# taqu/cpprcoder

Hardware: AMD Instinct MI355X
Metric: MB/s encode+decode per GPU on 64 KiB blocks; ratio vs CPU ref (higher is better)
Workload: dtype u32

## Files before the change

cpprcoder_amd/csrc/rcx_lane.hpp:

```cpp
#pragma once
#include <stdint.h>

#if defined(__HIPCC__)
#define RCX_DEV __device__ __forceinline__
#define RCX_HD __host__ __device__ inline
#else
#define RCX_HD inline
#define RCX_DEV inline
#define RCX_HOST_SIM 1
#endif

typedef uint8_t u8;
typedef uint32_t u32;
typedef uint64_t u64;
typedef int32_t s32;

struct alignas(16) U4 {
    u32 x, y, z, w;
};

#define RCX_LANES 64
#define RCX_G_L3 0
#define RCX_G_L2 1
#define RCX_G_L1 5
#define RCX_G_L0 21
#define RCX_GROUPS 85
#define RCX_STAGE 64
#define RCX_RING_DW 32
#define RCX_HALVE_AT (1u << 24)

struct alignas(16) DivEntry {
    u32 mul, add, shift, total;
};

#if defined(RCX_HOST_SIM)
RCX_DEV u32 rcx_clz(u32 x) { return (u32)__builtin_clz(x); }
RCX_DEV u32 rcx_mul24(u32 a, u32 b) { return (a & 0xFFFFFFu) * (b & 0xFFFFFFu); }
RCX_DEV u32 rcx_perm(u32 hi, u32 lo, u32 sel)
{
    u64 v = ((u64)hi << 32) | lo;
    u32 out = 0;
    for (int i = 0; i < 4; ++i) out |= (u32)((v >> (8 * ((sel >> (8 * i)) & 7))) & 0xFF) << (8 * i);
    return out;
}
RCX_DEV u32 rcx_bswap(u32 x) { return __builtin_bswap32(x); }
RCX_DEV void rcx_lds_inc(u32* p) { *p += 1; }
#if defined(RCX_SIM_RCP)
RCX_DEV float rcx_rcp(float x) { return RCX_SIM_RCP(1.0f / x); }
#else
RCX_DEV float rcx_rcp(float x) { return 1.0f / x; }
#endif
RCX_DEV bool rcx_any(bool p) { return p; }
RCX_DEV u32 rcx_funnel_shr(u32 hi, u32 lo, u32 sh) { return (u32)(((((u64)hi) << 32) | lo) >> (sh & 31u)); }
#define RCX_COLD inline
extern uint64_t rcx_sim_counters[4];
#define RCX_SIM_COUNT(i, n) (rcx_sim_counters[i] += (n))
#else
#define RCX_SIM_COUNT(i, n) ((void)0)
RCX_DEV u32 rcx_clz(u32 x) { return (u32)__builtin_clz(x); }
RCX_DEV u32 rcx_mul24(u32 a, u32 b) { return __umul24(a, b); }
RCX_DEV u32 rcx_perm(u32 hi, u32 lo, u32 sel) { return __builtin_amdgcn_perm(hi, lo, sel); }
RCX_DEV u32 rcx_bswap(u32 x) { return __builtin_bswap32(x); }
RCX_DEV void rcx_lds_inc(u32* p) { (void)__hip_atomic_fetch_add(p, 1u, __ATOMIC_RELAXED, __HIP_MEMORY_SCOPE_WAVEFRONT); }
RCX_DEV void rcx_lds_add(u32* p, u32 v) { (void)__hip_atomic_fetch_add(p, v, __ATOMIC_RELAXED, __HIP_MEMORY_SCOPE_WAVEFRONT); }
RCX_DEV float rcx_rcp(float x) { return __builtin_amdgcn_rcpf(x); }
RCX_DEV bool rcx_any(bool p) { return __builtin_expect(__any(p) != 0, 0); }
RCX_DEV u32 rcx_funnel_shr(u32 hi, u32 lo, u32 sh) { return __builtin_amdgcn_alignbit(hi, lo, sh); }
#define RCX_COLD __device__ __attribute__((noinline, cold))
#endif

RCX_DEV u32 rcx_div(u32 n, const DivEntry& k) { return (u32)(((u64)n * k.mul + k.add) >> 32) >> k.shift; }

#if !defined(RCX_TREE_PLANAR)
#define RCX_TREE_PLANAR 0
#endif
struct Tree {
    u32* col;
#if RCX_TREE_PLANAR
    RCX_DEV u32* at(u32 g, u32 p) const { return col + (4 * g + p) * RCX_LANES; }
    RCX_DEV U4 group(u32 g) const
    {
        const u32* a = col + 4 * g * RCX_LANES;
        U4 v;
        v.x = a[0];
        v.y = a[RCX_LANES];
        v.z = a[2 * RCX_LANES];
        v.w = a[3 * RCX_LANES];
        return v;
    }
    RCX_DEV void store(u32 g, const U4& v) const
    {
        u32* a = col + 4 * g * RCX_LANES;
        a[0] = v.x;
        a[RCX_LANES] = v.y;
        a[2 * RCX_LANES] = v.z;
        a[3 * RCX_LANES] = v.w;
    }
#else
    RCX_DEV u32* at(u32 g, u32 p) const { return col + 4 * g * RCX_LANES + p; }
    RCX_DEV U4 group(u32 g) const { return *reinterpret_cast<const U4*>(col + 4 * g * RCX_LANES); }
    RCX_DEV void store(u32 g, const U4& v) const { *reinterpret_cast<U4*>(col + 4 * g * RCX_LANES) = v; }
#endif
    RCX_DEV void bump(u32 g, u32 p) const { rcx_lds_inc(at(g, p)); }
    RCX_DEV void put(u32 g, u32 p, u32 value) const { *at(g, p) = value; }
    RCX_DEV void reset() const
    {
        U4 v;
        v.x = v.y = v.z = v.w = 64;
        store(RCX_G_L3, v);
        v.x = v.y = v.z = v.w = 16;
        for (u32 g = RCX_G_L2; g < RCX_G_L1; ++g) store(g, v);
        v.x = v.y = v.z = v.w = 4;
        for (u32 g = RCX_G_L1; g < RCX_G_L0; ++g) store(g, v);
// ... 122 lines not shown
        base = wave_base;
        off = slot_off + 4;
        cap = (slot_bytes - 4) & ~3u;
        reset_state();
    }

    RCX_DEV void idle(u8* wave_base)
    {
        base = wave_base;
        off = 0;
        cap = 0;
        reset_state();
        leader = false;
    }

    RCX_DEV void carry_into_memory(u32 extra) { rcx_carry_walk(base + off, leader ? (pos < cap ? pos : 0u) : 0u, extra); }

    RCX_DEV void track(u32 index, u32 carry, u32 moved, u32 k8)
    {
        if (trk_fail_at != 0xFFFFFFFFu) return;
        if (carry && trk_pending > 0) {
            if (trk_written + trk_pending > trk_cap) { trk_fail_at = index; return; }
            trk_written += trk_pending;
            trk_pending = 0;
        }
        for (u32 s = 0; s < k8; s += 8) {
            if (((moved << s) >> 24) != 0xFFu) {
                if (trk_written + 1 + trk_pending > trk_cap) { trk_fail_at = index; return; }
                trk_written += 1 + trk_pending;
                trk_pending = 0;
            } else {
                trk_pending += 1;
            }
        }
    }
    RCX_DEV bool track_flush_fails() const { return trk_written + 1 + trk_pending > trk_cap; }

    template <bool WIDE = false>
    RCX_DEV u32 arith(u32 cum, u32 f, const DivEntry& k)
    {
        return arith_t<WIDE>(cum, f, rcx_div(range, k));
    }
    template <bool WIDE = false>
    RCX_DEV u32 arith_t(u32 cum, u32 f, u32 t)
    {
        const u32 moved = low + (WIDE ? cum * t : rcx_mul24(cum, t));
        const u32 carry = moved < low ? 1u : 0u;
        range = WIDE ? f * t : rcx_mul24(f, t);
        const u32 k8 = rcx_clz(range) & 0x18u;
        low = moved << k8;
        range <<= k8;
        return (moved & 0xFFFFFF00u) | k8 | carry;
    }
    RCX_DEV u32 arith_q(u32 cum, u32 f, u32 mul, u32 shift, u64 add)
    {
        const u32 t = (u32)(((u64)range * mul + add) >> 32) >> (shift & 31u);
        const u32 moved = low + rcx_mul24(cum, t);
        const u32 carry = moved < low ? 1u : 0u;
        range = rcx_mul24(f, t);
        const u32 k8 = rcx_clz(range) & 0x18u;
        low = moved << k8;
        range <<= k8;
        return (moved & 0xFFFFFF00u) | k8 | carry;
    }
    RCX_DEV void emit(u32 rec)
    {
        const u32 k8 = rec & 0x18u;
        acc += rec & 1u;
        acc = (acc << k8) | (((u64)rec << k8) >> 32);
        nacc8 += k8;
        flush();
    }
    template <bool TRACK = false, bool WIDE = false>
    RCX_DEV void code(u32 cum, u32 f, const DivEntry& k, u32 index = 0)
    {
        const u32 rec = arith<WIDE>(cum, f, k);
        if (TRACK) track(index, rec & 1u, rec & 0xFFFFFF00u, rec & 0x18u);
        emit(rec);
    }

    RCX_DEV void flush()
    {
        const bool due = nacc8 >= 40;
        const u32 keep8 = (nacc8 - 32) & 31u;
        const u32 acc_lo = (u32)acc, acc_hi = (u32)(acc >> 32);
        const u32 word = rcx_funnel_shr(acc_hi, acc_lo, keep8);
        const u32 extra = due ? acc_hi >> keep8 : 0u;
        if (rcx_any(extra != 0)) rcx_carry_slow(base + off, leader ? (pos < cap ? pos : 0u) : 0u, extra);
        const u32 where = pos < cap - 4 ? pos : cap - 4;
        if (due && leader) *reinterpret_cast<u32*>(base + (off + where)) = rcx_bswap(word);
        const u32 kept = acc_lo & ((1u << keep8) - 1u);
        acc = due ? (u64)kept : acc;
        nacc8 -= due ? 32u : 0u;
        pos += due ? 4u : 0u;
    }
    template <bool TRACK = false, class TreeT>
    RCX_DEV void step(const TreeT& tree, u32 c, const DivEntry& k, u32 index = 0)
    {
        const U4 g3 = tree.group(RCX_G_L3);
        const U4 g2 = tree.group(RCX_G_L2 + (c >> 6));
        const U4 g1 = tree.group(RCX_G_L1 + (c >> 4));
        const U4 g0 = tree.group(RCX_G_L0 + (c >> 2));
        const u32 cum = rcx_pre4(g3, c >> 6) + rcx_pre4(g2, (c >> 4) & 3) + rcx_pre4(g1, (c >> 2) & 3) + rcx_pre4(g0, c & 3);
        const u32 f = rcx_sel4(g0, c & 3);
        code<TRACK>(cum, f, k, index);
        tree.update(c);
    }

    template <bool TRACK = false, class TreeT>
    RCX_DEV void step_long(const TreeT& tree, u32 c, u32& total, u32 index = 0)
    {
        const U4 g3 = tree.group(RCX_G_L3);
        const U4 g2 = tree.group(RCX_G_L2 + (c >> 6));
        const U4 g1 = tree.group(RCX_G_L1 + (c >> 4));
        const U4 g0 = tree.group(RCX_G_L0 + (c >> 2));
// ... 319 lines not shown
```

cpprcoder_amd/csrc/rcx_launch.hpp:

```cpp
#pragma once
#include "rcx_ctx.hpp"

namespace
{

bool wide_workgroups(const rcx_ctx* c, u64 nblocks)
{
    (void)nblocks;
    return c->wide_wg != 0;
}

int decode_lanes(const rcx_ctx* c, u64 nblocks)
{
    (void)nblocks;
    return c->lanes_per_block ? c->lanes_per_block : 4;
}

u32 pow2_at_least(u64 x)
{
    u32 p = 1;
    while (p < x) p <<= 1;
    return p;
}
u32 encode_lanes(const rcx_ctx* c, u64 nblocks)
// ... 20 lines not shown
    u32* models;
    u32* redo;
};

template <class G>
int encode_launches(rcx_ctx* c, int coder, const void* d_src, u64 n, u32 block, u64 nblocks, ScratchView v, u64 slot, hipStream_t s, bool packed, G g)
{
    const u8* const src = static_cast<const u8*>(d_src);
    const int variant = (G::items && c->enc_variant != 0) ? 3 : c->enc_variant;
    const bool static3 = coder == RCX_CODER_STATIC && variant >= 2 && nblocks < 32768;
    auto adaptive_pass = [&](const u32* redo) {
        hipLaunchKernelGGL((rcx_enc_adaptive_k<false, false, G>), dim3(grid_for(nblocks, RCX_LANES)), dim3(64), 0, s, src, n, block, nblocks, v.slots,
                           slot, v.sizes, c->divtab(), c->status, 0u, static_cast<u32*>(nullptr), redo, g);
    };
    auto static_pass = [&](const u32* redo) {
        hipLaunchKernelGGL(rcx_enc_static_k<G>, dim3(grid_for(nblocks, RCX_LANES)), dim3(64), 0, s, src, n, block, nblocks, v.slots, slot, v.sizes,
                           c->status, redo, g);
    };
    Timed t(c, s, RCX_T_ENCODE);
    if (is_rans(coder)) {
        const u32 grid = grid_for(nblocks, 4 * RCX_RANS_BLOCKS);
        if (coder == RCX_CODER_RANS8)
            hipLaunchKernelGGL((rcx_enc_rans_k<true, G>), dim3(grid), dim3(256), 0, s, src, n, block, nblocks, v.slots, slot, v.sizes, v.starts,
                               c->status, g);
        else {
            hipLaunchKernelGGL((rcx_rans_model_k<14, G>), dim3(grid), dim3(256), 0, s, src, n, block, nblocks, v.models, g);
            const char* one = getenv("RCX_RANS1_WAVES");
            if (!(one && atoi(one) == 1)) {
                if (allow_lds(c, &rcx_enc_rans1w_k<G>, RCX_R1W_LDS_BYTES) != RCX_OK) return RCX_E_HIP;
                hipLaunchKernelGGL(rcx_enc_rans1w_k<G>, dim3(grid_for(nblocks, 64)), dim3(128), RCX_R1W_LDS_BYTES, s, src, n, block, nblocks,
                                   static_cast<const u32*>(v.models), v.slots, slot, v.sizes, v.starts, c->status, g);
            } else {
                u32 lanes = 16;
                if (const char* v2 = getenv("RCX_RANS1_LANES")) { const int q = atoi(v2); if (q == 1 || q == 2 || q == 4 || q == 8 || q == 16) lanes = (u32)q; }
                u32 lds_bytes = lanes * RCX_RANS1_ENC_WAVES * 2048u;
                if (getenv("RCX_RANS1_ALONE") && lds_bytes < 84u * 1024u) lds_bytes = 84u * 1024u;
                u32 lanes_shift = 0;
                while ((1u << lanes_shift) < lanes) ++lanes_shift;
                if (allow_lds(c, &rcx_enc_rans1_k<G>, 128 * 1024) != RCX_OK) return RCX_E_HIP;
                hipLaunchKernelGGL(rcx_enc_rans1_k<G>, dim3(grid_for(nblocks, (u64)lanes * RCX_RANS1_ENC_WAVES)), dim3(64 * RCX_RANS1_ENC_WAVES), lds_bytes,
                                   s, src, n, block, nblocks, static_cast<const u32*>(v.models), v.slots, slot, v.sizes, v.starts, c->status, lanes_shift, g);
            }
        }
    } else if (static3) {
        const u32 lanes = packed ? RCX_LANES : encode_lanes(c, nblocks);
        hipLaunchKernelGGL(rcx_enc_static3_k<G>, dim3(grid_for(nblocks, lanes)), dim3(RCX_ST3_THREADS), 0, s, src, n, block, nblocks, v.slots, slot,
                           v.sizes, c->status, v.redo, lanes, g);
        static_pass(v.redo);
    } else if (coder == RCX_CODER_STATIC) {
        static_pass(nullptr);
    } else if (variant == 3) {
        const u32 lanes = packed ? RCX_LANES : encode_lanes(c, nblocks);
        hipLaunchKernelGGL(rcx_enc_mc5_k<G>, dim3(grid_for(nblocks, lanes)), dim3(RCX_MC5_THREADS), 0, s, src, n, block, nblocks, v.slots, slot,
                           v.sizes, c->divtab(), c->status, v.redo, lanes, g);
        adaptive_pass(v.redo);
#if defined(RCX_WITH_VARIANTS)
    } else if (variant == 2) {
        hipLaunchKernelGGL(rcx_enc_mc_k, dim3(grid_for(nblocks, RCX_LANES)), dim3(RCX_MC_THREADS), 0, s, src, n, block, nblocks, v.slots, slot,
                           v.sizes, c->divtab(), c->status);
    } else if (variant == 1) {
        hipLaunchKernelGGL(rcx_enc_oct_k, dim3(grid_for(nblocks, RCX_OCT_BLOCKS)), dim3(64), 0, s, src, n, block, nblocks, v.slots, slot, v.sizes,
                           c->divtab(), c->status);
#endif
    } else {
        adaptive_pass(nullptr);
    }
    return RCX_OK;
}

int encode_range(rcx_ctx* c, int coder, const void* d_src, u64 n, u32 block, void* d_dst, u64 dst_cap, u64* d_offsets, hipStream_t s,
                 ScratchRange rg)
{
    const u64 nblocks = rcx_block_count(n, block);
    const u64 slot = rcx_block_bound_for(coder, block);
    ScratchView v{c->slots + rg.first * slot, c->sizes + rg.first, c->starts ? c->starts + rg.first : nullptr,
                  c->models ? c->models + rg.first * RCX_RANS_MODEL_DW : nullptr, c->redo + rg.first};
    {
        const int e = encode_launches(c, coder, d_src, n, block, nblocks, v, slot, s, rg.packed, RcxBlocks{});
        if (e != RCX_OK) return e;
    }
    {
        Timed t(c, s, RCX_T_SCAN);
        hipLaunchKernelGGL(rcx_scan_sizes_k, dim3(1), dim3(1024), 0, s, v.sizes, nblocks, d_offsets, dst_cap, c->status);
    }
    {
        Timed t(c, s, RCX_T_SCATTER);
        hipLaunchKernelGGL(rcx_scatter_k, dim3((u32)nblocks), dim3(256), 0, s, v.slots, slot, v.sizes, d_offsets,
                           static_cast<u8*>(d_dst), dst_cap, is_rans(coder) ? static_cast<const u32*>(v.starts) : static_cast<const u32*>(nullptr));
    }
    return LAUNCHED();
}

template <class G>
int decode_launches(rcx_ctx* c, int coder, const void* d_comp, u64 comp_size, const u64* d_offsets, u64 nblocks, u32 block, u64 n, void* d_dst,
                    hipStream_t s, u32* redo, bool packed, G g)
{
    const u8* const comp = static_cast<const u8*>(d_comp);
    u8* const dst = static_cast<u8*>(d_dst);
    const int lanes_per = (G::items && decode_lanes(c, nblocks) == 8) ? 4 : decode_lanes(c, nblocks);
    const u32 quads = packed ? RCX_QUAD_BLOCKS : decode_quads(c, nblocks);
    const u32 quad_grid = grid_for(nblocks, (u64)quads * RCX_QUAD_DEC_WAVES), quad_threads = 64 * RCX_QUAD_DEC_WAVES;
    auto adaptive_pass = [&](const u32* marks) {
        hipLaunchKernelGGL((rcx_dec_adaptive_k<false, false, G>), dim3(grid_for(nblocks, RCX_LANES)), dim3(64), 0, s, comp, comp_size, d_offsets, nblocks,
                           block, n, dst, c->divtab(), c->status, static_cast<u32*>(nullptr), marks, g);
    };
    auto static_pass = [&](const u32* marks) {
        hipLaunchKernelGGL((rcx_dec_static_k<false, G>), dim3(grid_for(nblocks, RCX_LANES)), dim3(64), 0, s, comp, comp_size, d_offsets, nblocks, block, n,
// ... 62 lines not shown
```

cpprcoder_amd/csrc/rcx_mc.hpp:

```cpp
#pragma once

#define RCX_MC_CHUNK 16
#define RCX_MC_THREADS 256
#define RCX_MC_RING_U4 (2 * RCX_MC_CHUNK * RCX_LANES)
#define RCX_MC_LDS_U4 (RCX_LDS_U4 + RCX_MC_RING_U4)

__device__ __forceinline__ void rcx_lds_barrier()
{
    asm volatile("s_waitcnt lgkmcnt(0)\n\ts_barrier" ::: "memory");
}

#if defined(RCX_STAMP)
static __device__ unsigned long long rcx_stamp_out[16];
#define rcx_stamp_wait stamp_wait_
#endif
struct alignas(16) DivQ {
    u32 mul, st;
    u64 add;
};

#define RCX_DRAIN_WAVE 5
#define RCX_L3_WAVE 6
#define RCX_MC5_THREADS 448
#define RCX_MC5_ROLE(HW) ((0x6541230u >> (4u * (HW))) & 15u)
#if !defined(RCX_RING_PLANAR)
#define RCX_RING_PLANAR 0
#endif
#if !defined(RCX_MODEL_AHEAD)
#define RCX_MODEL_AHEAD 2
#endif
#if !defined(RCX_ARITH_AHEAD)
#define RCX_ARITH_AHEAD 1
#endif
#if RCX_RING_PLANAR
#define RCX_RING_LANE 1
#define RCX_RING_AT(s, f) ((4 * (s) + (f)) * RCX_LANES)
#else
#define RCX_RING_LANE 4
#define RCX_RING_AT(s, f) (4 * (s) * RCX_LANES + (f))
#endif
#define RCX_MC5_RING2_DW (2 * RCX_MC_CHUNK * RCX_LANES)
#define RCX_OUT_RING_WORDS 64
#define RCX_OUT_MARGIN 32
#define RCX_MC5_OUT_DW (RCX_OUT_RING_WORDS * RCX_LANES + 3 * RCX_LANES)
#define RCX_MC5_RING3_DW (2 * RCX_MC_CHUNK * RCX_LANES)
#define RCX_MC5_LDS_U4 (RCX_MC_LDS_U4 + RCX_MC5_RING2_DW / 4 + RCX_LANES / 4 + RCX_MC5_OUT_DW / 4 + RCX_MC5_RING3_DW / 4)

struct __attribute__((packed, aligned(4))) RcxU4Unaligned {
    u32 x, y, z, w;
};

__device__ __attribute__((noinline, cold)) u32 rcx_stage_carry(u32* ring_lane, u32 pos, u32 safe_from, u32 extra)
{
    while (extra != 0 && pos > safe_from) {
        --pos;
        u32* w = ring_lane + ((pos >> 2) % RCX_OUT_RING_WORDS) * RCX_LANES;
        const u32 sh = 8u * (pos & 3u);
        const u32 old = *w;
        const u32 v = ((old >> sh) & 0xFFu) + extra;
        *w = (old & ~(0xFFu << sh)) | ((v & 0xFFu) << sh);
        extra = v >> 8;
    }
    return extra != 0 && pos != 0 ? 1u : 0u;
}

__device__ __attribute__((noinline, cold)) u32 rcx_stage_far_carry(u32* ring_lane, u64 acc_after, u32 pos8, u32 safe_from, u32 far)
{
    if (!far) return 0;
    const u64 before = acc_after - 1;
    const u32 sh8 = (0u - pos8) & 24u;
    const u64 t = before << sh8;
    const u32 w = (pos8 - 8u) >> 5;
    ring_lane[((w - 1u) % RCX_OUT_RING_WORDS) * RCX_LANES] = rcx_bswap((u32)(t >> 32));
    ring_lane[(w % RCX_OUT_RING_WORDS) * RCX_LANES] = rcx_bswap((u32)t);
    return rcx_stage_carry(ring_lane, pos8 >> 3, safe_from, 1u);
}

__device__ __attribute__((noinline, cold)) u32 rcx_drain_more(const u32* ring_lane, u8* payload, u32 drained, u32 lim, bool live)
{
    while (__any(live && drained + 16 <= lim)) {
        if (live && drained + 16 <= lim) {
            const u32* w = ring_lane + ((drained >> 2) % RCX_OUT_RING_WORDS) * RCX_LANES;
            RcxU4Unaligned piece;
            piece.x = w[0];
            piece.y = w[RCX_LANES];
            piece.z = w[2 * RCX_LANES];
            piece.w = w[3 * RCX_LANES];
            *reinterpret_cast<RcxU4Unaligned*>(payload + drained) = piece;
            drained += 16;
        }
    }
    return drained;
}
__device__ __forceinline__ u32 rcx_drain_piece(const u32* ring_lane, u8* payload, u32 drained, u32 lim, bool live, const RcxU4Unaligned& piece)
{
    const bool go = live && drained + 16 <= lim;
    {
        const u64 lanes = __ballot(go);
        u8* at = payload + drained;
// ... 97 lines not shown
#define RCX_MC_WRITER_STAGE(K, RING2, WR, OUT_POS)                                                                     \
    if ((K) >= 2) {                                                                                                    \
        const u32* rs2 = (RING2) + (((K)-2) & 1u) * (RCX_MC_CHUNK * RCX_LANES) + lane;                                 \
        u32 ra_next = rs2[0], rb_next = rs2[RCX_LANES];                                                                \
        (WR).chunk_begins();                                                                                           \
        _Pragma("unroll") for (u32 s = 0; s < RCX_MC_CHUNK; s += 2)                                                    \
        {                                                                                                              \
            const u32 ra = ra_next, rb = rb_next;                                                                      \
            if (s + 2 < RCX_MC_CHUNK) ra_next = rs2[(s + 2) * RCX_LANES], rb_next = rs2[(s + 3) * RCX_LANES];          \
            (WR).emit(ra);                                                                                             \
            (WR).emit(rb);                                                                                             \
        }                                                                                                              \
        (OUT_POS)[lane] = (WR).chunk_ends();                                                                           \
    }

#define RCX_MC_DRAIN_READ(P, PIECE, OUT_POS, WR, DRAINED)                                                              \
    {                                                                                                                  \
        P = (OUT_POS)[lane];                                                                                           \
        const u32* w = (WR).ring_lane + (((DRAINED) >> 2) % RCX_OUT_RING_WORDS) * RCX_LANES;  \
        PIECE.x = w[0];                                                                                                \
        PIECE.y = w[RCX_LANES];                                                                                        \
        PIECE.z = w[2 * RCX_LANES];                                                                                    \
        PIECE.w = w[3 * RCX_LANES];                                                                                    \
    }
#define RCX_MC_DRAIN_STORE(P, PIECE, WR, PAYLOAD, DRAINED, CAP, LIVE)                                                  \
    {                                                                                                                  \
        const u32 limit = (P) > RCX_OUT_MARGIN ? ((P)-RCX_OUT_MARGIN) & ~15u : 0u;                                     \
        DRAINED = rcx_drain_piece((WR).ring_lane, PAYLOAD, DRAINED, limit < (CAP) ? limit : (CAP), LIVE, PIECE);       \
    }

#define RCX_MC_CLOSE_HANDOVER(WAVE, DRAIN_WAVE, OUT, ENC, DRAINED)                                                     \
    if ((WAVE) == 0) OUT.final_low[lane] = (ENC).low;                                                                  \
    if ((WAVE) == (DRAIN_WAVE)) {                                                                                      \
        OUT.drained[lane] = DRAINED;                                                                                   \
        __builtin_amdgcn_s_waitcnt(0x0F70);                                                              \
    }                                                                                                                  \
    rcx_lds_barrier()
#define RCX_MC_CLOSE_FLUSH(OUT, WR, ENC, PAYLOAD, CAP)                                                                 \
    {                                                                                                                  \
        u32 at_ = OUT.drained[lane];                                                                                   \
        const u32 flushed = (WR).finish(ENC);                                                                          \
        const u32 end = flushed < (CAP) ? flushed : (CAP);                                                             \
        for (; at_ < end; at_ += 4)                                                                                    \
            *reinterpret_cast<u32*>((PAYLOAD) + at_) = (WR).ring_lane[((at_ >> 2) % RCX_OUT_RING_WORDS) * RCX_LANES];  \
        (ENC).low = OUT.final_low[lane];                                                                               \
    }
#define RCX_MC_CLOSE_REPORT(BYTES, ENC, WR, GEOM, BLK, SLOT, SIZES, STATUS, REDO)                                      \
    (SIZES)[BLK] = (ENC).overflow ? (u32)(SLOT) : (BYTES);                                                             \
    if ((ENC).overflow) rcx_flag(STATUS, RCX_ST_CAPACITY, rcx_id(GEOM, BLK));                                          \
    (REDO)[BLK] = ((WR).redo != 0 && !(ENC).overflow) ? 1u : 0u

template <bool FULL>
__device__ __forceinline__ void rcx_mc5_pipeline(u32 wave, u32 lane, u32 len, u32 nchunks, const u8* in,
                                                 const DivEntry* __restrict__ divtab, const Tree& tree, DivEntry* stage,
                                                 u32* ring, u32* ring2, u32* ring3, EncLane& enc, DivEntry& ahead, StagedWriter& wr,
                                                 u32* out_pos, u32& drained, u8* payload, u32 cap, bool live)
{
#if defined(RCX_STAMP)
    unsigned long long stamp_wait_ = 0;
    const unsigned long long stamp_begin_ = __builtin_amdgcn_s_memtime();
#endif
    if (wave == 4) __builtin_amdgcn_s_setprio(1);
    U4 piece_ahead;
    piece_ahead.x = piece_ahead.y = piece_ahead.z = piece_ahead.w = 0;
    if (FULL && wave >= 2 && wave != RCX_DRAIN_WAVE && nchunks > 0) piece_ahead = *reinterpret_cast<const U4*>(in);
    u32 l3a = 64, l3b = 128, l3c = 192;
    for (u32 k = 0; k <= nchunks + 1; ++k) {
        if (wave == 0) {
            if (k >= 1 && k <= nchunks) {
                const u32 i0 = (k - 1) * RCX_MC_CHUNK;
                if ((i0 % RCX_STAGE) == 0) {
                    DivQ q;
                    q.mul = ahead.mul;
                    q.st = ahead.shift;
                    q.add = ahead.add;
                    reinterpret_cast<DivQ*>(stage)[lane] = q;
                    ahead = divtab[i0 + RCX_STAGE + lane];
                }
                const u32* rs = ring + ((k - 1) & 1u) * (4 * RCX_MC_CHUNK * RCX_LANES) + RCX_RING_LANE * lane;
                const u32* rs3 = ring3 + ((k - 1) & 1u) * (RCX_MC_CHUNK * RCX_LANES) + lane;
                u32* ws2 = ring2 + ((k - 1) & 1u) * (RCX_MC_CHUNK * RCX_LANES) + lane;
                u32 st_lds = (u32)reinterpret_cast<uintptr_t>(stage + (i0 % RCX_STAGE));
                asm volatile("" : "+v"(st_lds));
                const RcxLdsDivQ* st = reinterpret_cast<const RcxLdsDivQ*>(st_lds);
                U4 eq[RCX_MC_CHUNK];
                u32 c3q[RCX_MC_CHUNK];
                RcxDivQv kq[RCX_MC_CHUNK];
                u32 rec_even = 0;
#define RCX_A_ISSUE(T)                                                                                              \
    {                                                                                                               \
        eq[T].x = rs[RCX_RING_AT((T), 0)], eq[T].y = rs[RCX_RING_AT((T), 1)], eq[T].z = rs[RCX_RING_AT((T), 2)];    \
        eq[T].w = rs[RCX_RING_AT((T), 3)];                                                                          \
        if (((T)&1u) == 0) c3q[T] = rs3[(T)*RCX_LANES], c3q[(T) + 1] = rs3[((T) + 1) * RCX_LANES];                   \
        kq[T] = st[T];                                                                                              \
    }
#pragma unroll
                for (u32 t = 0; t < RCX_ARITH_AHEAD; ++t) RCX_A_ISSUE(t);
#pragma unroll
                for (u32 s = 0; s < RCX_MC_CHUNK; ++s) {
                    if (s + RCX_ARITH_AHEAD < RCX_MC_CHUNK) RCX_A_ISSUE(s + RCX_ARITH_AHEAD);
                    const U4 e = eq[s];
                    const RcxDivQv kk = kq[s];
                    u32 rec = 0;
                    if (FULL || i0 + s < len) rec = enc.arith_q(e.x + e.y + e.z + c3q[s], e.w, kk.x, kk.y, ((u64)kk.w << 32) | kk.z);
                    if ((s & 1u) == 0) rec_even = rec;
                    else {
                        ws2[(s - 1) * RCX_LANES] = rec_even;
                        ws2[s * RCX_LANES] = rec;
                    }
                }
#undef RCX_A_ISSUE
            }
        } else if (wave == 1) {
            RCX_MC_WRITER_STAGE(k, ring2, wr, out_pos)
        } else if (wave == RCX_DRAIN_WAVE) {
            u32 drain_p;
            RcxU4Unaligned drain_piece;
            RCX_MC_DRAIN_READ(drain_p, drain_piece, out_pos, wr, drained)
            RCX_MC_DRAIN_STORE(drain_p, drain_piece, wr, payload, drained, cap, live)
        } else if (k < nchunks) {
            const u32 i0 = k * RCX_MC_CHUNK;
            u32* ws = ring + (k & 1u) * (4 * RCX_MC_CHUNK * RCX_LANES) + RCX_RING_LANE * lane;
            U4 piece;
            if (FULL) {
                piece = piece_ahead;
                if (k + 1 < nchunks) piece_ahead = *reinterpret_cast<const U4*>(in + i0 + RCX_MC_CHUNK);
            } else if (i0 + RCX_MC_CHUNK <= len && (reinterpret_cast<uintptr_t>(in) & 15u) == 0) {
                piece = *reinterpret_cast<const U4*>(in + i0);
            } else {
                u32 w[4] = {0, 0, 0, 0};
                for (u32 s = 0; s < RCX_MC_CHUNK; ++s)
                    if (i0 + s < len) w[s >> 2] |= (u32)in[i0 + s] << (8 * (s & 3));
                piece.x = w[0];
                piece.y = w[1];
                piece.z = w[2];
                piece.w = w[3];
            }
            U4 ga[RCX_MC_CHUNK], gb[RCX_MC_CHUNK];
            u32 held = 0, held_f = 0;
            if (wave == 2) {
#define RCX_M2_ISSUE(T)                                                       \
    {                                                                         \
        const u32 c_ = rcx_byte_of(piece, (T));                               \
        gb[T] = tree.group(RCX_G_L2 + (c_ >> 6));                             \
        if (FULL || i0 + (T) < len) tree.bump(RCX_G_L2 + (c_ >> 6), (c_ >> 4) & 3); \
    }
#pragma unroll
                for (u32 t = 0; t < RCX_MODEL_AHEAD; ++t) RCX_M2_ISSUE(t);
#pragma unroll
                for (u32 s = 0; s < RCX_MC_CHUNK; ++s) {
                    if (s + RCX_MODEL_AHEAD < RCX_MC_CHUNK) RCX_M2_ISSUE(s + RCX_MODEL_AHEAD);
                    const u32 cc = rcx_byte_of(piece, s);
                    const u32 sum32 = rcx_pre4(gb[s], (cc >> 4) & 3);
                    if (FULL) {
                        if ((s & 1u) == 0) held = sum32;
                        else ws[RCX_RING_AT(s - 1, 0)] = held, ws[RCX_RING_AT(s, 0)] = sum32;
                    } else if (i0 + s < len) ws[RCX_RING_AT(s, 0)] = sum32;
                }
#undef RCX_M2_ISSUE
            } else if (wave == 4) {
#define RCX_M1_ISSUE(T)                                                       \
    {                                                                         \
        const u32 c_ = rcx_byte_of(piece, (T));                               \
        ga[T] = tree.group(RCX_G_L1 + (c_ >> 4));                             \
        if (FULL || i0 + (T) < len) tree.bump(RCX_G_L1 + (c_ >> 4), (c_ >> 2) & 3); \
    }
// ... 10 lines not shown
                    } else if (i0 + s < len) ws[RCX_RING_AT(s, 1)] = sum1;
                }
#undef RCX_M1_ISSUE
            } else if (wave == RCX_L3_WAVE) {
                u32* ws3 = ring3 + (k & 1u) * (RCX_MC_CHUNK * RCX_LANES) + lane;
#pragma unroll
                for (u32 s = 0; s < RCX_MC_CHUNK; ++s) {
                    const u32 cc = rcx_byte_of(piece, s);
                    u32 cum3;
                    u64 m1_, m2_, m3_, cz_;
                    asm volatile("v_cmp_gt_u32_e64 %[m3], %[k192], %[c]\n\t"
                                 "v_cmp_gt_u32_e64 %[m2], %[k128], %[c]\n\t"
                                 "v_cmp_gt_u32_e64 %[m1], 64, %[c]\n\t"
                                 "v_cndmask_b32_e64 %[x], %[pc], %[pb], %[m3]\n\t"
                                 "v_cndmask_b32_e64 %[x], %[x], %[pa], %[m2]\n\t"
                                 "v_cndmask_b32_e64 %[x], %[x], 0, %[m1]\n\t"
                                 "v_addc_co_u32_e64 %[pc], %[cz], %[pc], 0, %[m3]\n\t"
                                 "v_addc_co_u32_e64 %[pb], %[cz], %[pb], 0, %[m2]\n\t"
                                 "v_addc_co_u32_e64 %[pa], %[cz], %[pa], 0, %[m1]"
                                 : [x] "=&v"(cum3), [pa] "+v"(l3a), [pb] "+v"(l3b), [pc] "+v"(l3c), [m1] "=&s"(m1_), [m2] "=&s"(m2_),
                                   [m3] "=&s"(m3_), [cz] "=&s"(cz_)
                                 : [c] "v"(cc), [k192] "s"(192u), [k128] "s"(128u));
                    if ((s & 1u) == 0) held = cum3;
                    else ws3[(s - 1) * RCX_LANES] = held, ws3[s * RCX_LANES] = cum3;
                }
            } else {
#define RCX_M0_ISSUE(T)                                                       \
    {                                                                         \
        const u32 c_ = rcx_byte_of(piece, (T));                               \
        ga[T] = tree.group(RCX_G_L0 + (c_ >> 2));                             \
        if (FULL || i0 + (T) < len) tree.bump(RCX_G_L0 + (c_ >> 2), c_ & 3);  \
    }
#pragma unroll
                for (u32 t = 0; t < RCX_MODEL_AHEAD; ++t) RCX_M0_ISSUE(t);
#pragma unroll
                for (u32 s = 0; s < RCX_MC_CHUNK; ++s) {
                    if (s + RCX_MODEL_AHEAD < RCX_MC_CHUNK) RCX_M0_ISSUE(s + RCX_MODEL_AHEAD);
                    const u32 cc = rcx_byte_of(piece, s);
                    const u32 sum0 = rcx_pre4(ga[s], cc & 3), f0 = rcx_sel4(ga[s], cc & 3);
                    if (FULL) {
                        if ((s & 1u) == 0) held = sum0, held_f = f0;
                        else {
                            ws[RCX_RING_AT(s - 1, 2)] = held, ws[RCX_RING_AT(s, 2)] = sum0;
                            ws[RCX_RING_AT(s - 1, 3)] = held_f, ws[RCX_RING_AT(s, 3)] = f0;
                        }
                    } else if (i0 + s < len) {
                        ws[RCX_RING_AT(s, 2)] = sum0;
                        ws[RCX_RING_AT(s, 3)] = f0;
                    }
                }
#undef RCX_M0_ISSUE
            }
        }
#if defined(RCX_STAMP)
        const unsigned long long t0_ = __builtin_amdgcn_s_memtime();
        rcx_lds_barrier();
        stamp_wait_ += __builtin_amdgcn_s_memtime() - t0_;
#else
        rcx_lds_barrier();
#endif
    }
#if defined(RCX_STAMP)
    if (blockIdx.x == 7 && lane == 0) {
        rcx_stamp_out[wave * 2] = __builtin_amdgcn_s_memtime() - stamp_begin_;
        rcx_stamp_out[wave * 2 + 1] = stamp_wait_;
    }
#endif
}

template <class G = RcxBlocks>
__global__ __launch_bounds__(RCX_MC5_THREADS) void rcx_enc_mc5_k(const u8* __restrict__ src, u64 n, u32 block, u64 nblocks,
                                                                u8* __restrict__ slots, u64 slot, u32* __restrict__ sizes,
                                                                const DivEntry* __restrict__ divtab, u32* status,
                                                                u32* __restrict__ redo, u32 lanes_used, const G g = G())
{
    __shared__ U4 lds[RCX_MC5_LDS_U4];
    const u32 lane = threadIdx.x & 63u;
    const u32 wave = RCX_MC5_ROLE(__builtin_amdgcn_readfirstlane(threadIdx.x >> 6));
    const bool in_use = lane < lanes_used;
    const u64 blk = in_use ? (u64)blockIdx.x * lanes_used + lane : nblocks;
    RCX_ENTRY(g, blk, nblocks, n, block);

    Tree tree{reinterpret_cast<u32*>(lds) + (RCX_TREE_PLANAR ? 1 : 4) * lane};
    DivEntry* stage = reinterpret_cast<DivEntry*>(lds + RCX_GROUPS * RCX_LANES);
    u32* ring = reinterpret_cast<u32*>(lds + RCX_LDS_U4);
    u32* ring2 = reinterpret_cast<u32*>(lds + RCX_MC_LDS_U4);
    RCX_MC_OUTPUT(oq, ring2 + RCX_MC5_RING2_DW);
    u32* ring3 = oq.drained + RCX_LANES;

    const u32 maxlen = rcx_wave_max(len);
    bool full;
    if constexpr (G::items) {
        full = __all((!in_use || (live && len == maxlen)) && ((reinterpret_cast<uintptr_t>(src) + at) & 15u) == 0) && (maxlen % 16u == 0);
    } else {
        full = __all(!in_use || (live && len == block)) && (block % 16u == 0) && ((reinterpret_cast<uintptr_t>(src) & 15u) == 0);
    }
    const u8* in = src + at;
    const u32 nchunks = (maxlen + RCX_MC_CHUNK - 1) / RCX_MC_CHUNK;

    EncLane enc;
    u8* wave_slots = slots + (u64)blockIdx.x * lanes_used * slot;
    enc.idle(wave_slots);
    StagedWriter wr;
    wr.begin(oq.ring, oq.dummy, lane);
    u32 drained = 0;
    DivEntry ahead;
    ahead.mul = ahead.add = ahead.shift = ahead.total = 0;
    U4 v;
    if (wave == 0) {
        ahead = divtab[lane];
    } else if (wave == 1) {
        if (live) enc.begin(wave_slots, lane * (u32)slot, (u32)slot, len);
        oq.pos[lane] = 0;
    } else if (wave == 2) {
        v.x = v.y = v.z = v.w = 16;
        for (u32 g = RCX_G_L2; g < RCX_G_L1; ++g) tree.store(g, v);
    } else if (wave == 4) {
        v.x = v.y = v.z = v.w = 4;
        for (u32 g = RCX_G_L1; g < RCX_G_L0; ++g) tree.store(g, v);
    } else if (wave == 3) {
        v.x = v.y = v.z = v.w = 1;
        for (u32 g = RCX_G_L0; g < RCX_GROUPS; ++g) tree.store(g, v);
    }
    rcx_lds_barrier();

    u8* payload = wave_slots + (u64)lane * slot + 4;
    const u32 cap = ((u32)slot - 4) & ~3u;
    if (full) rcx_mc5_pipeline<true>(wave, lane, len, nchunks, in, divtab, tree, stage, ring, ring2, ring3, enc, ahead, wr, oq.pos, drained, payload, cap, live);
    else rcx_mc5_pipeline<false>(wave, lane, len, nchunks, in, divtab, tree, stage, ring, ring2, ring3, enc, ahead, wr, oq.pos, drained, payload, cap, live);

    RCX_MC_CLOSE_HANDOVER(wave, RCX_DRAIN_WAVE, oq, enc, drained);
    if (wave == 1 && live) {
        RCX_MC_CLOSE_FLUSH(oq, wr, enc, payload, cap)
        const u32 bytes = enc.finish();
        RCX_MC_CLOSE_REPORT(bytes, enc, wr, g, blk, slot, sizes, status, redo);
    } else if (wave == 1 && blk < nblocks) {
        redo[blk] = 0;
    }
}
```

cpprcoder_amd/csrc/rcx_streams.hpp:

```cpp
#pragma once
#include "rcx_launch.hpp"

#define RCX_DSTREAM_CHUNK (1u << 20)

struct rcx_dstream {
    rcx_ctx* ctx = nullptr;
    DevBuf<RcxDState> state;
    DevBuf<u8> in;
    u64 in_base = 0;
    u64 in_bytes = 0;
    u64 consumed = 0;
    DevBuf<u8> out;
    DevBuf<u32> result;
    PinBuf<u32> result_host;
    bool finished = false;
    u32 declared = 0, produced = 0;
};

struct rcx_estream {
    rcx_ctx* ctx = nullptr;
    DevBuf<RcxEState> state;
    DevBuf<RcxEState> backup;
    DevBuf<u8> slot;
    u64 slot_bytes = 0;
// ... 72 lines not shown
                      uint8_t* dst, uint64_t dst_cap, uint64_t sink_capacity, uint64_t* dst_size, uint32_t* request_size)
{
    if (!c || !dst || !dst_size || (n && !src)) return RCX_E_ARG;
    if (!coder_ok(coder) || n > RCX_MAX_STREAM) return RCX_E_ARG;
    HIP_TRY(rcx_enter_device(c->device));
    *dst_size = 0;
    if (request_size) *request_size = 0;
    const u32 block = n < RCX_MIN_BLOCK ? RCX_MIN_BLOCK : n;
    if (is_rans(coder)) {
        if (n == 0 || n > RCX_MAX_RANS_STREAM) return RCX_ERROR;
        int rr = reserve(c, block, block, coder);
        if (rr == RCX_OK) rr = stage_source(c, src, n);
        if (rr != RCX_OK) return rr;
        const u64 rslot = rcx_block_bound_for(coder, block);
        if (coder == RCX_CODER_RANS8)
            hipLaunchKernelGGL(rcx_enc_rans_k<true>, dim3(1), dim3(256), 0, nullptr, c->h_in, (u64)n, block, (u64)1, c->slots, rslot, c->sizes,
                               c->starts, c->status);
        else
            hipLaunchKernelGGL(rcx_enc_rans_k<false>, dim3(1), dim3(256), 0, nullptr, c->h_in, (u64)n, block, (u64)1, c->slots, rslot, c->sizes,
                               c->starts, c->status);
        return fetch_stream(c, c->starts, dst, dst_cap, sink_capacity, dst_size);
    }
    const bool longer = n > RCX_MAX_BLOCK;
    const u64 slot = rcx_block_bound(block);
    int r = longer ? RCX_OK : ensure_divtab(c, block);
    if (r == RCX_OK) r = c->slots.reserve(slot + 256);
    if (r == RCX_OK) r = c->sizes.reserve(2);
    if (r == RCX_OK) r = stage_source(c, src, n);
    if (r != RCX_OK) return r;
    auto adaptive_pass = [&](const u32* redo) {
        hipLaunchKernelGGL((rcx_enc_adaptive_k<false, false>), dim3(1), dim3(64), 0, nullptr, c->h_in, (u64)n, block, (u64)1, c->slots, slot,
                           c->sizes, c->divtab(), c->status, 0u, static_cast<u32*>(nullptr), redo);
    };
    auto static_pass = [&](const u32* redo) {
        hipLaunchKernelGGL(rcx_enc_static_k, dim3(1), dim3(64), 0, nullptr, c->h_in, (u64)n, block, (u64)1, c->slots, slot, c->sizes, c->status, redo);
    };
    if (coder == RCX_CODER_STATIC) {
        if (c->enc_variant >= 2 && n >= RCX_MIN_BLOCK && n <= RCX_MAX_BLOCK) {
            if ((r = ensure_redo(c, 1)) != RCX_OK) return r;
            hipLaunchKernelGGL(rcx_enc_static3_k, dim3(1), dim3(RCX_ST3_THREADS), 0, nullptr, c->h_in, (u64)n, block, (u64)1, c->slots, slot,
                               c->sizes, c->status, c->redo, 1u);
            static_pass(c->redo);
        } else {
            static_pass(nullptr);
        }
        return fetch_stream(c, nullptr, dst, dst_cap, sink_capacity, dst_size);
    }
    if (longer) {
        hipLaunchKernelGGL((rcx_enc_adaptive_k<false, true>), dim3(1), dim3(64), 0, nullptr, c->h_in, (u64)n, block, (u64)1, c->slots, slot,
                           c->sizes, c->divtab(), c->status, 0u, static_cast<u32*>(nullptr), static_cast<const u32*>(nullptr));
    } else if (c->enc_variant == 3 && n >= RCX_MIN_BLOCK) {
        if ((r = ensure_redo(c, 1)) != RCX_OK) return r;
        hipLaunchKernelGGL(rcx_enc_mc5_k, dim3(1), dim3(RCX_MC5_THREADS), 0, nullptr, c->h_in, (u64)n, block, (u64)1, c->slots, slot, c->sizes,
                           c->divtab(), c->status, c->redo, 1u);
        adaptive_pass(c->redo);
    } else {
        adaptive_pass(nullptr);
    }
    HIP_TRY(hipGetLastError());
    r = rcx_ctx_sync_status(c, nullptr, nullptr);
    if (r != RCX_OK) return r;
    u32 size = 0;
    HIP_TRY(hipMemcpy(&size, c->sizes, sizeof(u32), hipMemcpyDeviceToHost));
    const u64 cap16 = sink_capacity < 4 ? 4 : sink_capacity;
    if ((u64)size - 4 <= cap16) {
        *dst_size = size;
        if (size > dst_cap) return RCX_E_CAPACITY;
        HIP_TRY(hipMemcpy(dst, c->slots, size, hipMemcpyDeviceToHost));
        return RCX_OK;
    }
    *dst_size = cap16;
    if (cap16 > dst_cap) return RCX_E_CAPACITY;
    if (longer)
        hipLaunchKernelGGL((rcx_enc_adaptive_k<true, true>), dim3(1), dim3(64), 0, nullptr, c->h_in, (u64)n, block, (u64)1, c->slots, slot,
                           c->sizes, c->divtab(), c->status, (u32)(cap16 - 4), c->status + 2, static_cast<const u32*>(nullptr));
    else
        hipLaunchKernelGGL((rcx_enc_adaptive_k<true, false>), dim3(1), dim3(64), 0, nullptr, c->h_in, (u64)n, block, (u64)1, c->slots, slot,
                           c->sizes, c->divtab(), c->status, (u32)(cap16 - 4), c->status + 2, static_cast<const u32*>(nullptr));
    HIP_TRY(hipGetLastError());
    HIP_TRY(hipMemcpy(c->status_host, c->status, 4 * sizeof(u32), hipMemcpyDeviceToHost));
    const u32 fail_at = c->status_host[2];
    HIP_TRY(hipMemcpy(dst, c->slots, cap16, hipMemcpyDeviceToHost));
    if (fail_at != 0xFFFFFFFFu) {
        if (request_size) *request_size = n - fail_at;
        return RCX_PENDING;
    }
    return RCX_OK;
}

int rcx_stream_decode(rcx_ctx* c, int coder, const uint8_t* comp, uint64_t comp_size,
                      uint8_t* dst, uint64_t sink_capacity, uint64_t* dst_size, uint32_t* request_size)
{
    if (!c || !dst || !dst_size || (comp_size && !comp)) return RCX_E_ARG;
    if (!coder_ok(coder) || comp_size > 0xFFFFFFFFull) return RCX_E_ARG;
    HIP_TRY(rcx_enter_device(c->device));
    *dst_size = 0;
    if (request_size) *request_size = 0;
    if (is_rans(coder)) {
        if (comp_size < 1032 + 4) return RCX_ERROR;
        const u32 declared = le32(comp);
        if (declared > sink_capacity || declared == 0 || declared > RCX_MAX_RANS_STREAM) return RCX_ERROR;
        const u32 rblock = declared < RCX_MIN_BLOCK ? RCX_MIN_BLOCK : declared;
        int rr = stage_stream(c, comp, comp_size, declared);
        if (rr != RCX_OK) return rr;
        c->rans_track = true;
        rr = rcx_decode_blocks_device(c, coder, c->h_in, comp_size, c->h_off, 1, rblock, declared, c->h_out, nullptr);
        c->rans_track = false;
// ... 283 lines not shown
```

Measured before the change: 79050.

## Replace LDS-staged division table with register-held per-quad divisor constants in mc5 encoder

The arithmetic wave of the mc5 encoder used to stage 64-bit-add DivQ entries through shared memory each 64 symbols and read them back per symbol. It now loads compact multiplier/increment words per chunk straight from a new divq table into registers. The division uses mulhi with a shift derived from clz of the symbol index, and the range renormalisation shift is folded into the next step. Wave 0 is split out of the shared step loop into its own loop, and role/priority maps become configurable macros. This is meant to cut LDS traffic and 64-bit arithmetic on the critical serial wave. It depends on c->divq() and RCX_QUAD_DIVQ_DW being defined elsewhere, and the barrier count in wave 0's loop must stay matched with the other waves.

```diff
diff --git a/cpprcoder_amd/csrc/rcx_lane.hpp b/cpprcoder_amd/csrc/rcx_lane.hpp
--- a/cpprcoder_amd/csrc/rcx_lane.hpp
+++ b/cpprcoder_amd/csrc/rcx_lane.hpp
@@ -36,6 +36,7 @@
 #if defined(RCX_HOST_SIM)
 RCX_DEV u32 rcx_clz(u32 x) { return (u32)__builtin_clz(x); }
 RCX_DEV u32 rcx_mul24(u32 a, u32 b) { return (a & 0xFFFFFFu) * (b & 0xFFFFFFu); }
+RCX_DEV u32 rcx_mulhi(u32 a, u32 b) { return (u32)(((u64)a * b) >> 32); }
 RCX_DEV u32 rcx_perm(u32 hi, u32 lo, u32 sel)
 {
     u64 v = ((u64)hi << 32) | lo;
@@ -59,6 +60,7 @@
 #define RCX_SIM_COUNT(i, n) ((void)0)
 RCX_DEV u32 rcx_clz(u32 x) { return (u32)__builtin_clz(x); }
 RCX_DEV u32 rcx_mul24(u32 a, u32 b) { return __umul24(a, b); }
+RCX_DEV u32 rcx_mulhi(u32 a, u32 b) { return __umulhi(a, b); }
 RCX_DEV u32 rcx_perm(u32 hi, u32 lo, u32 sel) { return __builtin_amdgcn_perm(hi, lo, sel); }
 RCX_DEV u32 rcx_bswap(u32 x) { return __builtin_bswap32(x); }
 RCX_DEV void rcx_lds_inc(u32* p) { (void)__hip_atomic_fetch_add(p, 1u, __ATOMIC_RELAXED, __HIP_MEMORY_SCOPE_WAVEFRONT); }
@@ -287,15 +289,14 @@
         range <<= k8;
         return (moved & 0xFFFFFF00u) | k8 | carry;
     }
-    RCX_DEV u32 arith_q(u32 cum, u32 f, u32 mul, u32 shift, u64 add)
-    {
-        const u32 t = (u32)(((u64)range * mul + add) >> 32) >> (shift & 31u);
+    RCX_DEV u32 arith_i(u32 cum, u32 f, u32 mul, u32 inc, u32 sh, u32& k8)
+    {
+        const u32 t = rcx_mulhi((range << k8) + inc, mul) >> sh;
         const u32 moved = low + rcx_mul24(cum, t);
         const u32 carry = moved < low ? 1u : 0u;
         range = rcx_mul24(f, t);
-        const u32 k8 = rcx_clz(range) & 0x18u;
+        k8 = rcx_clz(range) & 0x18u;
         low = moved << k8;
-        range <<= k8;
         return (moved & 0xFFFFFF00u) | k8 | carry;
     }
     RCX_DEV void emit(u32 rec)
diff --git a/cpprcoder_amd/csrc/rcx_launch.hpp b/cpprcoder_amd/csrc/rcx_launch.hpp
--- a/cpprcoder_amd/csrc/rcx_launch.hpp
+++ b/cpprcoder_amd/csrc/rcx_launch.hpp
@@ -96,7 +96,7 @@
     } else if (variant == 3) {
         const u32 lanes = packed ? RCX_LANES : encode_lanes(c, nblocks);
         hipLaunchKernelGGL(rcx_enc_mc5_k<G>, dim3(grid_for(nblocks, lanes)), dim3(RCX_MC5_THREADS), 0, s, src, n, block, nblocks, v.slots, slot,
-                           v.sizes, c->divtab(), c->status, v.redo, lanes, g);
+                           v.sizes, c->divq(), c->status, v.redo, lanes, g);
         adaptive_pass(v.redo);
 #if defined(RCX_WITH_VARIANTS)
     } else if (variant == 2) {
diff --git a/cpprcoder_amd/csrc/rcx_mc.hpp b/cpprcoder_amd/csrc/rcx_mc.hpp
--- a/cpprcoder_amd/csrc/rcx_mc.hpp
+++ b/cpprcoder_amd/csrc/rcx_mc.hpp
@@ -14,15 +14,17 @@
 static __device__ unsigned long long rcx_stamp_out[16];
 #define rcx_stamp_wait stamp_wait_
 #endif
-struct alignas(16) DivQ {
-    u32 mul, st;
-    u64 add;
-};
 
 #define RCX_DRAIN_WAVE 5
 #define RCX_L3_WAVE 6
 #define RCX_MC5_THREADS 448
-#define RCX_MC5_ROLE(HW) ((0x6541230u >> (4u * (HW))) & 15u)
+#if !defined(RCX_MC5_ROLES)
+#define RCX_MC5_ROLES 0x6541230u
+#endif
+#if !defined(RCX_MC5_PRIO)
+#define RCX_MC5_PRIO 0x10u
+#endif
+#define RCX_MC5_ROLE(HW) (((u32)RCX_MC5_ROLES >> (4u * (HW))) & 15u)
 #if !defined(RCX_RING_PLANAR)
 #define RCX_RING_PLANAR 0
 #endif
@@ -44,7 +46,8 @@
 #define RCX_OUT_MARGIN 32
 #define RCX_MC5_OUT_DW (RCX_OUT_RING_WORDS * RCX_LANES + 3 * RCX_LANES)
 #define RCX_MC5_RING3_DW (2 * RCX_MC_CHUNK * RCX_LANES)
-#define RCX_MC5_LDS_U4 (RCX_MC_LDS_U4 + RCX_MC5_RING2_DW / 4 + RCX_LANES / 4 + RCX_MC5_OUT_DW / 4 + RCX_MC5_RING3_DW / 4)
+#define RCX_MC5_TREE_U4 (RCX_GROUPS * RCX_LANES)
+#define RCX_MC5_LDS_U4 (RCX_MC5_TREE_U4 + RCX_MC_RING_U4 + RCX_MC5_RING2_DW / 4 + RCX_LANES / 4 + RCX_MC5_OUT_DW / 4 + RCX_MC5_RING3_DW / 4)
 
 struct __attribute__((packed, aligned(4))) RcxU4Unaligned {
     u32 x, y, z, w;
@@ -248,47 +251,59 @@
 
 template <bool FULL>
 __device__ __forceinline__ void rcx_mc5_pipeline(u32 wave, u32 lane, u32 len, u32 nchunks, const u8* in,
-                                                 const DivEntry* __restrict__ divtab, const Tree& tree, DivEntry* stage,
-                                                 u32* ring, u32* ring2, u32* ring3, EncLane& enc, DivEntry& ahead, StagedWriter& wr,
+                                                 const u32* __restrict__ divq, const Tree& tree,
+                                                 u32* ring, u32* ring2, u32* ring3, EncLane& enc, StagedWriter& wr,
                                                  u32* out_pos, u32& drained, u8* payload, u32 cap, bool live)
 {
 #if defined(RCX_STAMP)
     unsigned long long stamp_wait_ = 0;
     const unsigned long long stamp_begin_ = __builtin_amdgcn_s_memtime();
-#endif
-    if (wave == 4) __builtin_amdgcn_s_setprio(1);
-    U4 piece_ahead;
-    piece_ahead.x = piece_ahead.y = piece_ahead.z = piece_ahead.w = 0;
-    if (FULL && wave >= 2 && wave != RCX_DRAIN_WAVE && nchunks > 0) piece_ahead = *reinterpret_cast<const U4*>(in);
-    u32 l3a = 64, l3b = 128, l3c = 192;
-    for (u32 k = 0; k <= nchunks + 1; ++k) {
-        if (wave == 0) {
-            if (k >= 1 && k <= nchunks) {
+#define RCX_MC5_STEP_ENDS()                                                \
+    {                                                                      \
+        const unsigned long long t0_ = __builtin_amdgcn_s_memtime();       \
+        rcx_lds_barrier();                                                 \
+        stamp_wait_ += __builtin_amdgcn_s_memtime() - t0_;                 \
+    }
+#define RCX_MC5_STAMPS_OUT()                                               \
+    if (blockIdx.x == 7 && lane == 0) {                                    \
+        rcx_stamp_out[wave * 2] = __builtin_amdgcn_s_memtime() - stamp_begin_; \
+        rcx_stamp_out[wave * 2 + 1] = stamp_wait_;                         \
+    }
+#else
+#define RCX_MC5_STEP_ENDS() rcx_lds_barrier()
+#define RCX_MC5_STAMPS_OUT()
+#endif
+    if ((RCX_MC5_PRIO >> wave) & 1u) __builtin_amdgcn_s_setprio(1);
+    if (wave == 0) {
+        U4 dm[4], di[4];
+        u32 prev_k8 = 0;
+        u32 vz;
+        asm volatile("v_mov_b32 %0, 0" : "=v"(vz));
+        const u32* dq = divq + vz;
+#pragma unroll
+        for (u32 q = 0; q < 4; ++q) {
+            dm[q] = reinterpret_cast<const U4*>(dq)[q];
+            di[q] = reinterpret_cast<const U4*>(dq + 16)[q];
+        }
+        RCX_MC5_STEP_ENDS();
+        for (u32 k = 1; k <= nchunks; ++k) {
+            {
                 const u32 i0 = (k - 1) * RCX_MC_CHUNK;
-                if ((i0 % RCX_STAGE) == 0) {
-                    DivQ q;
-                    q.mul = ahead.mul;
-                    q.st = ahead.shift;
-                    q.add = ahead.add;
-                    reinterpret_cast<DivQ*>(stage)[lane] = q;
-                    ahead = divtab[i0 + RCX_STAGE + lane];
-                }
+                asm volatile("" ::"v"(dm[0].x), "v"(di[0].x), "v"(dm[1].x), "v"(di[1].x), "v"(dm[2].x), "v"(di[2].x), "v"(dm[3].x), "v"(di[3].x));
+                const u32 sh = 31u - rcx_clz(256u + i0);
+                const u32* dq_next = dq + (size_t)k * RCX_QUAD_DIVQ_DW;
                 const u32* rs = ring + ((k - 1) & 1u) * (4 * RCX_MC_CHUNK * RCX_LANES) + RCX_RING_LANE * lane;
                 const u32* rs3 = ring3 + ((k - 1) & 1u) * (RCX_MC_CHUNK * RCX_LANES) + lane;
                 u32* ws2 = ring2 + ((k - 1) & 1u) * (RCX_MC_CHUNK * RCX_LANES) + lane;
-                u32 st_lds = (u32)reinterpret_cast<uintptr_t>(stage + (i0 % RCX_STAGE));
-                asm volatile("" : "+v"(st_lds));
-                const RcxLdsDivQ* st = reinterpret_cast<const RcxLdsDivQ*>(st_lds);
                 U4 eq[RCX_MC_CHUNK];
                 u32 c3q[RCX_MC_CHUNK];
-                RcxDivQv kq[RCX_MC_CHUNK];
                 u32 rec_even = 0;
+#define RCX_A_U4_AT(V, C) ((C) == 0 ? (V).x : (C) == 1 ? (V).y : (C) == 2 ? (V).z : (V).w)
 #define RCX_A_ISSUE(T)                                                                                              \
     {                                                                                                               \
         eq[T].x = rs[RCX_RING_AT((T), 0)], eq[T].y = rs[RCX_RING_AT((T), 1)], eq[T].z = rs[RCX_RING_AT((T), 2)];    \
         eq[T].w = rs[RCX_RING_AT((T), 3)];                                                                          \
         if (((T)&1u) == 0) c3q[T] = rs3[(T)*RCX_LANES], c3q[(T) + 1] = rs3[((T) + 1) * RCX_LANES];                   \
-        kq[T] = st[T];                                                                                              \
     }
 #pragma unroll
                 for (u32 t = 0; t < RCX_ARITH_AHEAD; ++t) RCX_A_ISSUE(t);
@@ -296,9 +311,15 @@
                 for (u32 s = 0; s < RCX_MC_CHUNK; ++s) {
                     if (s + RCX_ARITH_AHEAD < RCX_MC_CHUNK) RCX_A_ISSUE(s + RCX_ARITH_AHEAD);
                     const U4 e = eq[s];
-                    const RcxDivQv kk = kq[s];
                     u32 rec = 0;
-                    if (FULL || i0 + s < len) rec = enc.arith_q(e.x + e.y + e.z + c3q[s], e.w, kk.x, kk.y, ((u64)kk.w << 32) | kk.z);
+                    if (FULL || i0 + s < len)
+                        rec = enc.arith_i(e.x + e.y + e.z + c3q[s], e.w, RCX_A_U4_AT(dm[s >> 2], s & 3u), RCX_A_U4_AT(di[s >> 2], s & 3u), sh, prev_k8);
+                    if ((s & 3u) == 3u) {
+                        asm volatile("" ::: "memory");
+                        dm[s >> 2] = reinterpret_cast<const U4*>(dq_next)[s >> 2];
+                        di[s >> 2] = reinterpret_cast<const U4*>(dq_next + 16)[s >> 2];
+                        asm volatile("" ::: "memory");
+                    }
                     if ((s & 1u) == 0) rec_even = rec;
                     else {
                         ws2[(s - 1) * RCX_LANES] = rec_even;
@@ -306,8 +327,20 @@
                     }
                 }
 #undef RCX_A_ISSUE
+#undef RCX_A_U4_AT
             }
-        } else if (wave == 1) {
+            RCX_MC5_STEP_ENDS();
+        }
+        RCX_MC5_STEP_ENDS();
+        RCX_MC5_STAMPS_OUT();
+        return;
+    }
+    U4 piece_ahead;
+    piece_ahead.x = piece_ahead.y = piece_ahead.z = piece_ahead.w = 0;
+    if (FULL && wave >= 2 && wave != RCX_DRAIN_WAVE && nchunks > 0) piece_ahead = *reinterpret_cast<const U4*>(in);
+    u32 l3a = 64, l3b = 128, l3c = 192;
+    for (u32 k = 0; k <= nchunks + 1; ++k) {
+        if (wave == 1) {
             RCX_MC_WRITER_STAGE(k, ring2, wr, out_pos)
         } else if (wave == RCX_DRAIN_WAVE) {
             u32 drain_p;
@@ -424,26 +457,17 @@
 #undef RCX_M0_ISSUE
             }
         }
-#if defined(RCX_STAMP)
-        const unsigned long long t0_ = __builtin_amdgcn_s_memtime();
-        rcx_lds_barrier();
-        stamp_wait_ += __builtin_amdgcn_s_memtime() - t0_;
-#else
-        rcx_lds_barrier();
-#endif
-    }
-#if defined(RCX_STAMP)
-    if (blockIdx.x == 7 && lane == 0) {
-        rcx_stamp_out[wave * 2] = __builtin_amdgcn_s_memtime() - stamp_begin_;
-        rcx_stamp_out[wave * 2 + 1] = stamp_wait_;
-    }
-#endif
+        RCX_MC5_STEP_ENDS();
+    }
+    RCX_MC5_STAMPS_OUT();
+#undef RCX_MC5_STEP_ENDS
+#undef RCX_MC5_STAMPS_OUT
 }
 
 template <class G = RcxBlocks>
 __global__ __launch_bounds__(RCX_MC5_THREADS) void rcx_enc_mc5_k(const u8* __restrict__ src, u64 n, u32 block, u64 nblocks,
                                                                 u8* __restrict__ slots, u64 slot, u32* __restrict__ sizes,
-                                                                const DivEntry* __restrict__ divtab, u32* status,
+                                                                const u32* __restrict__ divq, u32* status,
                                                                 u32* __restrict__ redo, u32 lanes_used, const G g = G())
 {
     __shared__ U4 lds[RCX_MC5_LDS_U4];
@@ -454,9 +478,8 @@
     RCX_ENTRY(g, blk, nblocks, n, block);
 
     Tree tree{reinterpret_cast<u32*>(lds) + (RCX_TREE_PLANAR ? 1 : 4) * lane};
-    DivEntry* stage = reinterpret_cast<DivEntry*>(lds + RCX_GROUPS * RCX_LANES);
-    u32* ring = reinterpret_cast<u32*>(lds + RCX_LDS_U4);
-    u32* ring2 = reinterpret_cast<u32*>(lds + RCX_MC_LDS_U4);
+    u32* ring = reinterpret_cast<u32*>(lds + RCX_MC5_TREE_U4);
+    u32* ring2 = reinterpret_cast<u32*>(lds + RCX_MC5_TREE_U4 + RCX_MC_RING_U4);
     RCX_MC_OUTPUT(oq, ring2 + RCX_MC5_RING2_DW);
     u32* ring3 = oq.drained + RCX_LANES;
 
@@ -476,12 +499,8 @@
     StagedWriter wr;
     wr.begin(oq.ring, oq.dummy, lane);
     u32 drained = 0;
-    DivEntry ahead;
-    ahead.mul = ahead.add = ahead.shift = ahead.total = 0;
     U4 v;
-    if (wave == 0) {
-        ahead = divtab[lane];
-    } else if (wave == 1) {
+    if (wave == 1) {
         if (live) enc.begin(wave_slots, lane * (u32)slot, (u32)slot, len);
         oq.pos[lane] = 0;
     } else if (wave == 2) {
@@ -498,8 +517,8 @@
 
     u8* payload = wave_slots + (u64)lane * slot + 4;
     const u32 cap = ((u32)slot - 4) & ~3u;
-    if (full) rcx_mc5_pipeline<true>(wave, lane, len, nchunks, in, divtab, tree, stage, ring, ring2, ring3, enc, ahead, wr, oq.pos, drained, payload, cap, live);
-    else rcx_mc5_pipeline<false>(wave, lane, len, nchunks, in, divtab, tree, stage, ring, ring2, ring3, enc, ahead, wr, oq.pos, drained, payload, cap, live);
+    if (full) rcx_mc5_pipeline<true>(wave, lane, len, nchunks, in, divq, tree, ring, ring2, ring3, enc, wr, oq.pos, drained, payload, cap, live);
+    else rcx_mc5_pipeline<false>(wave, lane, len, nchunks, in, divq, tree, ring, ring2, ring3, enc, wr, oq.pos, drained, payload, cap, live);
 
     RCX_MC_CLOSE_HANDOVER(wave, RCX_DRAIN_WAVE, oq, enc, drained);
     if (wave == 1 && live) {
diff --git a/cpprcoder_amd/csrc/rcx_streams.hpp b/cpprcoder_amd/csrc/rcx_streams.hpp
--- a/cpprcoder_amd/csrc/rcx_streams.hpp
+++ b/cpprcoder_amd/csrc/rcx_streams.hpp
@@ -148,7 +148,7 @@
     } else if (c->enc_variant == 3 && n >= RCX_MIN_BLOCK) {
         if ((r = ensure_redo(c, 1)) != RCX_OK) return r;
         hipLaunchKernelGGL(rcx_enc_mc5_k, dim3(1), dim3(RCX_MC5_THREADS), 0, nullptr, c->h_in, (u64)n, block, (u64)1, c->slots, slot, c->sizes,
-                           c->divtab(), c->status, c->redo, 1u);
+                           c->divq(), c->status, c->redo, 1u);
         adaptive_pass(c->redo);
     } else {
         adaptive_pass(nullptr);
```

New measurement: 82530, median of 6. +4.4%, better.
